# ZenHKD/ocr-vi-invoice

Measured on AMD Instinct MI355X. Metric: invoice images/sec end-to-end (det+rec), higher is better.
Workload: dtype f16x2

## Files before the change

include/ocrvi.h:

```cpp
#ifndef OCRVI_H
#define OCRVI_H

#include <stddef.h>
#include <stdint.h>

#ifdef __cplusplus
extern "C" {
#endif

#define OCRVI_OK 0
#define OCRVI_EINVAL (-1)
#define OCRVI_EHIP (-2)
#define OCRVI_ENOMEM (-3)
#define OCRVI_EBLOB (-4)
#define OCRVI_ERANGE (-5)

typedef enum { OCRVI_F32 = 0, OCRVI_BF16 = 1, OCRVI_F16 = 2, OCRVI_F16X2 = 3 } ocrvi_dtype;

const char* ocrvi_last_error(void);
int ocrvi_abi_version(void);

typedef struct ocrvi_det ocrvi_det;

typedef struct {
// ... 277 lines not shown
int ocrvi_test_gconv_plan(int dtype, int N, int C, int H, int W, int Co, int sh, int sw, int groups, int out_f32, int has_res, int n_cu,
                          int32_t plan[12]);
int ocrvi_test_conv3_halo_raw(int device, const float* x, const float* weight_host, const float* bias_host, int N, int C, int H, int W, int Co,
                              int act, void* out_raw, float* out);
int ocrvi_test_bneck_tail_raw(int device, const float* t1, const float* identity, const float* w2_host, const float* b2_host,
                              const float* w3_host, const float* b3_host, const float* w1_host, const float* b1_host, int N, int H, int W,
                              int no_phase_c, void* y_raw, void* t1n_raw, float* y_out, float* t1n_out);
int ocrvi_test_stem_pool_raw(int device, int dtype, const float* x, const float* weight_host, const float* bias_host, int N, int H, int W,
                             int fused, void* out_raw, float* out);
int ocrvi_test_halo_plan(int kind, int N, int C, int H, int W, int Co, int n_cu, int32_t plan[8]);
int ocrvi_test_stem_pool(int device, int dtype, const float* x, const float* weight_host, const float* bias_host, int N, int H, int W, int fused,
                         float* out, int iters, float* avg_ms);
int ocrvi_test_attention(int device, int dtype, const float* qkv, int B, int N, int heads, float* out, int iters,
                         float* avg_ms);

int ocrvi_test_mlp(int device, int dtype, float* x, const float* ln_g_host, const float* ln_b_host, const float* w1_host, const float* b1_host,
                   const float* w2_host, const float* b2_host, const float* next_g_host, const float* next_b_host, int want_xn, int M, int D,
                   float* xn_out, int iters, float* avg_ms);
int ocrvi_test_mlp_raw(int device, int dtype, float* x, const float* ln_g_host, const float* ln_b_host, const float* w1_host, const float* b1_host,
                       const float* w2_host, const float* b2_host, const float* next_g_host, const float* next_b_host, int M, int D, void* xn_raw,
                       float* xn_out, int iters, float* avg_ms);
int ocrvi_test_lin_x2(int device, const float* a, const float* weight_host, const float* bias_host, int M, int K, int N, int max_workgroups,
                      void* out_raw, float* out, int iters, float* avg_ms);
int ocrvi_test_pack_f16x2(const float* src, size_t n, void* dst, float* wscale);
int ocrvi_test_pack_stream(int kind, const float* w0, const float* w1, int d0, int d1, void* out, size_t cap, size_t* size, float scales[2]);
int ocrvi_test_swizzles(int32_t swz128_rows[64], int32_t swz_halo_rows[64]);
int ocrvi_test_persistent_grid(int ntile, int slots, int32_t* grid);

int ocrvi_test_layernorm(int device, int dtype, const float* x, int x_f32, int out_f32, const float* gamma_host, const float* beta_host,
                         int rows, int D, float* out);
int ocrvi_test_frm_vertical(int device, int dtype, const float* kv, const float* vq_host, int B, int H, int W, int D, float* out);
int ocrvi_test_asf(int device, int dtype, const float* p2, const float* p3, const float* p4, const float* p5, const float* w_host,
                   const float* b_host, int N, int H, int W, float* out);
int ocrvi_test_maxpool(int device, int dtype, const float* x, int N, int C, int H, int W, float* out);
int ocrvi_test_db_maps(int device, const float* bin_logits, const float* thresh_logits, float k, float* binary, float* thresh,
                       float* thresh_binary, size_t n);
int ocrvi_test_ctc_logsoftmax(int device, const float* logits, int ld, int B, int T, int C, float* log_probs, int32_t* argmax_ids);
int ocrvi_test_ctc_logsoftmax_conf(int device, const float* logits, int ld, int B, int T, int C, float* log_probs, int32_t* argmax_ids,
                                   float* best_lp);

int ocrvi_document_contour(const uint8_t* mask, int h, int w, int64_t stride, int32_t* quad , int32_t* found);
int ocrvi_document_contour_bits(const uint32_t* bits, int h, int w, int32_t* quad , int32_t* found);

#define OCRVI_DOC_AUTO 0
#define OCRVI_DOC_BRIGHT 1
#define OCRVI_DOC_DARK 2
// ... 31 lines not shown
```

ocr_vi_invoice_amd/_lib.py:

```python
from __future__ import annotations

import ctypes as C
import os
from typing import Optional

_HERE = os.path.dirname(os.path.abspath(__file__))
LIB_PATH = os.environ.get("OCRVI_LIB") or os.path.join(_HERE, "lib", "libocrvi.so")

OCRVI_F32, OCRVI_BF16, OCRVI_F16, OCRVI_F16X2 = 0, 1, 2, 3
DTYPES = {"f32": OCRVI_F32, "fp32": OCRVI_F32, "float32": OCRVI_F32, "bf16": OCRVI_BF16, "bfloat16": OCRVI_BF16,
          "f16": OCRVI_F16, "fp16": OCRVI_F16, "float16": OCRVI_F16,
          "f16x2": OCRVI_F16X2}
ABI_VERSION = 5

EXPORTS = [
    "ocrvi_last_error", "ocrvi_abi_version",
    "ocrvi_det_create", "ocrvi_det_destroy", "ocrvi_det_workspace_bytes", "ocrvi_det_forward", "ocrvi_det_debug_features",
    "ocrvi_rec_create", "ocrvi_rec_destroy", "ocrvi_rec_workspace_bytes", "ocrvi_rec_forward", "ocrvi_rec_debug_features",
    "ocrvi_ctc_greedy", "ocrvi_normalize_u8", "ocrvi_resize_u8", "ocrvi_crop_resize_normalize", "ocrvi_db_postprocess", "ocrvi_db_boxes_batch",
    "ocrvi_unclip_polygon", "ocrvi_db_components_workspace_bytes", "ocrvi_db_components", "ocrvi_db_boxes_batch_sparse",
    "ocrvi_test_deform_conv", "ocrvi_test_offset_conv", "ocrvi_test_conv", "ocrvi_test_gemm", "ocrvi_test_attention", "ocrvi_test_mlp", "ocrvi_test_stem_pool", "ocrvi_test_pack_f16x2",
    "ocrvi_prof_enable", "ocrvi_prof_reset", "ocrvi_prof_report",
    "ocrvi_det_status", "ocrvi_rec_status", "ocrvi_range_reset", "ocrvi_range_flag",
    "ocrvi_resize_normalize_pages", "ocrvi_crop_resize_normalize_pages", "ocrvi_db_boxes_pages",
# ... 4 lines not shown
    "ocrvi_test_deform_conv_res",
    "ocrvi_enhance_init", "ocrvi_enhance_tables", "ocrvi_enhance_workspace_bytes", "ocrvi_enhance_u8",
    "ocrvi_rgb_to_lab_u8", "ocrvi_lab_to_rgb_u8", "ocrvi_clahe_lab_u8", "ocrvi_nlm_lab_u8", "ocrvi_sharpen_u8",
    "ocrvi_min_area_quads", "ocrvi_quad_crops", "ocrvi_crop_quad_resize_normalize_pages", "ocrvi_crop_quad_resize_normalize",
    "ocrvi_jpeg_info", "ocrvi_jpeg_parse", "ocrvi_jpeg_table_entry", "ocrvi_jpeg_decode_pages",
    "ocrvi_test_conv_res", "ocrvi_test_db_tail",
    "ocrvi_db_target_jobs", "ocrvi_db_target_maps", "ocrvi_resize_normalize_pad_pages",
    "ocrvi_test_mlp_raw", "ocrvi_test_lin_x2", "ocrvi_test_pack_stream", "ocrvi_test_swizzles", "ocrvi_test_persistent_grid",
    "ocrvi_test_bneck_tail",
    "ocrvi_jpeg_quant_tables", "ocrvi_jpeg_encode_header", "ocrvi_jpeg_encode_sizes", "ocrvi_jpeg_encode_table_entry", "ocrvi_jpeg_encode_pages",
    "ocrvi_test_gemm_raw", "ocrvi_test_ring_plan",
    "ocrvi_overlay_segments", "ocrvi_overlay_pages",
    "ocrvi_test_deform_conv_raw", "ocrvi_test_dcn_plan",
    "ocrvi_test_conv_raw", "ocrvi_test_gconv_plan",
    "ocrvi_png_info", "ocrvi_png_parse", "ocrvi_png_table_entry", "ocrvi_png_plan", "ocrvi_png_decode_pages",
    "ocrvi_png_encode_sizes", "ocrvi_png_encode_table_entry", "ocrvi_png_encode_pages", "ocrvi_test_png_code_lengths",
    "ocrvi_document_contour", "ocrvi_document_contour_bits", "ocrvi_doc_working_size", "ocrvi_doc_mask_sizes", "ocrvi_doc_mask_pages",
    "ocrvi_doc_grey_u8", "ocrvi_doc_smooth_u8", "ocrvi_doc_histogram", "ocrvi_doc_otsu", "ocrvi_doc_mask_bits",
    "ocrvi_rec_forward_conf", "ocrvi_ctc_greedy_conf", "ocrvi_test_ctc_logsoftmax_conf",
    "ocrvi_test_conv3_halo_raw", "ocrvi_test_bneck_tail_raw", "ocrvi_test_stem_pool_raw", "ocrvi_test_halo_plan",
    "ocrvi_ctc_beam_workspace_bytes", "ocrvi_ctc_beam",
    "ocrvi_lm_build", "ocrvi_lm_score", "ocrvi_lm_create", "ocrvi_lm_destroy", "ocrvi_ctc_beam_lm_workspace_bytes", "ocrvi_ctc_beam_lm",
    "ocrvi_skew_sizes", "ocrvi_skew_scores_pages", "ocrvi_skew_edges_u8", "ocrvi_skew_scores", "ocrvi_skew_pick", "ocrvi_skew_quad",
]
PAGE_ENTRY = 4
DET_EVAL_RECORD_BYTES = 104
DET_EVAL_INT_SLOTS = ("tp", "fp", "fn", "positive_count", "negatives", "negative_count")
DET_EVAL_F64_SLOTS = ("pos_bce", "topk_bce", "dice_inter", "pred_mask", "gt_mask", "l1_num", "thresh_mask")
CTC_LOSS_MAX_TARGET = 1024
EDIT_DISTANCE_MAX_LEN = 2048
CTC_BEAM_MAX = 64
CTC_BEAM_MAX_T = 1024
LM_MAX_ORDER = 6
CLAHE_WORKSPACE_BYTES = 16384
ENHANCE_MIN_SIDE = 16
DB_TARGET_GT, DB_TARGET_MASK, DB_TARGET_THRESH = 0, 1, 2
DB_TARGET_JOB = 8
DB_TARGET_MAX_SIDE = 16384
JPEG_ENTRY = 64
PNG_ENTRY = 16
JPEG_ENC_ENTRY = 64
JPEG_HEADER_MAX = 640
PNG_ENC_ENTRY = 16
PNG_ENC_BLOCK = 16384
OVERLAY_SEG = 8
OVERLAY_PRIM = 8
# ... 79 lines not shown
    lib.ocrvi_four_point_transform.argtypes = [vp, vp, vp, i32p, i32p]
    lib.ocrvi_warp_perspective_u8.argtypes = [i32, vp, i32, i32, vp, vp, i32, i32, vp]
    lib.ocrvi_warp_perspective_pages.argtypes = [i32, vp, vp, vp, i32, vp]
    lib.ocrvi_db_boxes_pages.argtypes = [vp, i32, i32, i32, C.c_float, C.c_float, i32, C.c_float, C.c_float, vp, vp, vp, vp, vp,
                                         vp, i32, vp, vp, vp, i32, vp, vp, i32]
    lib.ocrvi_test_deform_conv.argtypes = [i32, i32, f32p, f32p, f32p, vp, vp, i32, i32, i32, i32, i32, i32, i32, f32p, i32,
                                           C.POINTER(C.c_float)]
    lib.ocrvi_test_deform_conv_res.argtypes = [i32, i32, f32p, f32p, f32p, vp, vp, f32p, i32, i32, i32, i32, i32, i32, i32, f32p, i32,
                                               C.POINTER(C.c_float)]
    lib.ocrvi_test_offset_conv.argtypes = [i32, i32, f32p, vp, vp, i32, i32, i32, i32, i32, f32p, i32, C.POINTER(C.c_float)]
    lib.ocrvi_test_conv.argtypes = [i32, i32, f32p, vp, vp, i32, i32, i32, i32, i32, i32, i32, i32, i32, i32, f32p, i32,
                                    C.POINTER(C.c_float)]
    lib.ocrvi_test_conv_res.argtypes = [i32, i32, f32p, vp, vp, f32p, i32, i32, i32, i32, i32, i32, i32, i32, f32p, i32, C.POINTER(C.c_float)]
    lib.ocrvi_test_bneck_tail.argtypes = [i32, f32p, f32p, vp, vp, vp, vp, vp, vp, i32, i32, i32, i32, f32p, f32p, i32, C.POINTER(C.c_float)]
    lib.ocrvi_test_db_tail.argtypes = [i32, i32, f32p, vp, vp, vp, vp, vp, vp, vp, vp, i32, i32, i32, i32, i32, f32p, f32p, i32,
                                       C.POINTER(C.c_float)]
    lib.ocrvi_test_gemm.argtypes = [i32, i32, f32p, vp, vp, f32p, i32, i32, i32, i32, i32, i32, f32p, i32, C.POINTER(C.c_float)]
    lib.ocrvi_test_gemm_raw.argtypes = [i32, i32, f32p, vp, vp, f32p, i32, i32, i32, i32, i32, i32, vp, f32p]
    lib.ocrvi_test_ring_plan.argtypes = [i32, i32, i32, i32, i32, i32, i32, i32, C.POINTER(C.c_int32)]
    lib.ocrvi_test_deform_conv_raw.argtypes = [i32, i32, f32p, f32p, f32p, vp, vp, f32p, i32, i32, i32, i32, i32, i32, i32, vp, f32p]
    lib.ocrvi_test_dcn_plan.argtypes = [i32, i32, i32, i32, i32, i32, i32, i32, C.POINTER(C.c_int32)]
    lib.ocrvi_test_conv_raw.argtypes = [i32, i32, f32p, vp, vp, f32p] + [i32] * 13 + [vp, f32p]
    lib.ocrvi_test_gconv_plan.argtypes = [i32] * 12 + [C.POINTER(C.c_int32)]
    lib.ocrvi_test_stem_pool.argtypes = [i32, i32, f32p, vp, vp, i32, i32, i32, i32, f32p, i32, C.POINTER(C.c_float)]
    lib.ocrvi_test_conv3_halo_raw.argtypes = [i32, f32p, vp, vp, i32, i32, i32, i32, i32, i32, vp, f32p]
    lib.ocrvi_test_bneck_tail_raw.argtypes = [i32, f32p, f32p, vp, vp, vp, vp, vp, vp, i32, i32, i32, i32, vp, vp, f32p, f32p]
    lib.ocrvi_test_stem_pool_raw.argtypes = [i32, i32, f32p, vp, vp, i32, i32, i32, i32, vp, f32p]
    lib.ocrvi_test_halo_plan.argtypes = [i32] * 7 + [C.POINTER(C.c_int32)]
    lib.ocrvi_test_attention.argtypes = [i32, i32, f32p, i32, i32, i32, f32p, i32, C.POINTER(C.c_float)]
    lib.ocrvi_test_mlp.argtypes = [i32, i32, f32p, vp, vp, vp, vp, vp, vp, vp, vp, i32, i32, i32, f32p, i32, C.POINTER(C.c_float)]
    lib.ocrvi_test_lin_x2.argtypes = [i32, f32p, vp, vp, i32, i32, i32, i32, vp, f32p, i32, C.POINTER(C.c_float)]
    lib.ocrvi_test_mlp_raw.argtypes = [i32, i32, f32p, vp, vp, vp, vp, vp, vp, vp, vp, i32, i32, vp, f32p, i32, C.POINTER(C.c_float)]
    lib.ocrvi_test_pack_f16x2.argtypes = [f32p, sz, vp, C.POINTER(C.c_float)]
    lib.ocrvi_test_pack_stream.argtypes = [i32, vp, vp, i32, i32, vp, sz, C.POINTER(sz), C.POINTER(C.c_float)]
    lib.ocrvi_test_swizzles.argtypes = [C.POINTER(C.c_int32), C.POINTER(C.c_int32)]
    lib.ocrvi_test_persistent_grid.argtypes = [i32, i32, C.POINTER(C.c_int32)]
    lib.ocrvi_test_layernorm.argtypes = [i32, i32, f32p, i32, i32, vp, vp, i32, i32, f32p]
    lib.ocrvi_test_frm_vertical.argtypes = [i32, i32, f32p, vp, i32, i32, i32, i32, f32p]
    lib.ocrvi_test_asf.argtypes = [i32, i32, f32p, f32p, f32p, f32p, vp, vp, i32, i32, i32, f32p]
    lib.ocrvi_test_maxpool.argtypes = [i32, i32, f32p, i32, i32, i32, i32, f32p]
    lib.ocrvi_test_db_maps.argtypes = [i32, f32p, f32p, C.c_float, f32p, f32p, f32p, sz]
    lib.ocrvi_test_ctc_logsoftmax.argtypes = [i32, f32p, i32, i32, i32, i32, f32p, i32p]
    lib.ocrvi_det_eval_workspace_bytes.argtypes = [i32, i32, i32, C.POINTER(sz)]
    lib.ocrvi_det_eval.argtypes = [i32, f32p, f32p, f32p, f32p, f32p, f32p, f32p, f32p, i32, i32, i32, C.c_double, vp, vp, sz, vp]
    lib.ocrvi_ctc_loss.argtypes = [i32, f32p, i32, i32, i32, i32p, i32, i32p, i32p, i32, vp, vp]
    lib.ocrvi_edit_distance.argtypes = [i32, i32p, i32, i32p, i32p, i32, i32p, i32, i32p, vp]
# ... 114 lines not shown
```

ocr_vi_invoice_amd/csrc/gconv32.h:

```cpp
#pragma once
#include "conv_gemm.h"

namespace ocrvi {

constexpr int GC_PS = 96;
constexpr int GC_TH = 4;
constexpr int GC_NBX = 5;

constexpr unsigned gc_hw_magic(int hw) { return 65536u / (unsigned)hw + 1; }
constexpr bool gc_hw_magic_exact() {
    for (int nbx = 1; nbx <= GC_NBX; ++nbx) {
        const int hw = 16 * nbx + 2;
        for (int pix = 0; pix < (GC_TH + 2) * hw; ++pix)
            if ((int)(((unsigned)pix * gc_hw_magic(hw)) >> 16) != pix / hw) return false;
    }
    return true;
}
static_assert(gc_hw_magic_exact(), "gconv32: the halo-index multiplication is not exact for every pixel of a (GC_TH + 2) x (16 GC_NBX + 2) tile");

template <typename T, bool F32O>
__global__ __launch_bounds__(256, 2) void gconv32_kernel(const ConvParams p, int TH, int nbx, int bands_y, int bands_x, unsigned hw_magic) {
    constexpr int PS = GC_PS, MB = (GC_TH * GC_NBX + 3) / 4;
    extern __shared__ __attribute__((aligned(16))) char smem[];
    const int tid = threadIdx.x, lane = tid & 63, wave = tid >> 6;
// ... 132 lines not shown
                if (F32O && p.res_mode == RES_SAME) {
                    const float4 rv = *(const float4*)((const float*)p.res + pix * p.ldr + ch);
                    v[nb][0] += rv.x; v[nb][1] += rv.y; v[nb][2] += rv.z; v[nb][3] += rv.w;
                }
                if (!p.res_post) activate(v[nb]);
                if (F32O) *(float4*)((float*)p.out + pix * p.ldo + p.out_coff + ch) = make_float4(v[nb][0], v[nb][1], v[nb][2], v[nb][3]);
            }
            if (!F32O) {
                union { T e[8]; uint4 u; } pk;
#pragma unroll
                for (int e = 0; e < 4; ++e) {
                    pk.e[e] = from_f32<T>(v[0][e]);
                    pk.e[4 + e] = from_f32<T>(v[1][e]);
                }
                *(uint4*)((T*)p.out + pix * p.ldo + p.out_coff + gp * 32 + 8 * g4) = pk.u;
            }
        }
        if (next >= ntile) break;
        tile = next;
        __syncthreads();
    }
}

static inline bool gconv32_eligible(const ConvParams& p, int amode, int esz) {
    static const bool on = !(getenv("OCRVI_GCONV32") && atoi(getenv("OCRVI_GCONV32")) == 0);
    if (!on || amode != AM_CONV3 || esz != 2 || p.groups < 2 || p.Cin_g != 32 || p.N_g != 32 || p.KH != 3) return false;
    if (p.SH != 1 || p.SW != 1 || p.PH != 1 || p.PW != 1 || p.H != p.OH || p.W != p.OW || p.store_mode != ST_NHWC) return false;
    if (p.Kp < 288 || p.Cin % 8 != 0 || p.cin_off % 8 != 0 || ((uintptr_t)p.x & 15) != 0 || ((uintptr_t)p.w & 15) != 0 || p.Kp % 8 != 0) return false;
    const int og = p.out_f32 ? 4 : 8;
    if (p.ldo % og != 0 || p.out_coff % og != 0 || ((uintptr_t)p.out & 15) != 0) return false;
    if (p.res_mode == RES_SAME) return p.out_f32 && p.res_f32 && p.ldr % 4 == 0 && ((uintptr_t)p.res & 15) == 0;
    return p.res_mode == RES_NONE;
}

struct Gconv32Plan {
    int th, nbx;
    int bands_y, bands_x;
    int ntile, grid_x;
    int tiles_min, tiles_max;
    int smem;
    unsigned hw_magic;
};
inline Gconv32Plan gconv32_plan(int n_img, int H, int W, int groups, int n_cu) {
    Gconv32Plan r;
    r.nbx = std::min(GC_NBX, cdiv(W, 16));
    r.th = H % 4 == 0 ? 4 : (H % 3 == 0 ? 3 : (H < 4 ? H : 4));
    r.bands_x = cdiv(W, 16 * r.nbx);
    r.bands_y = cdiv(H, r.th);
// ... 32 lines not shown
```

ocr_vi_invoice_amd/csrc/kernels.h:

```cpp
#pragma once
#include "common.h"

namespace ocrvi {

int k_nchw3_to_nhwc4_pad(int dtype, const float* x, void* y, int N, int H, int W, int pad_t, int pad_l, int Hp, int Wp, hipStream_t s);
int k_maxpool3x3s2(int dtype, const void* x, void* y, int N, int H, int W, int C, hipStream_t s);
bool stem_pool_eligible(int dtype, int cout, int Kp, int KH, int H, int W);
int k_stem_pool(int dtype, const void* xpad, const void* w, const float* bias, float wscale, void* y, int N, int H, int W, int Hp, int Wp,
                hipStream_t s);
struct StemPoolPlan {
    int tyN, txN, total;
    int grid;
    int tiles_min, tiles_max;
};
StemPoolPlan stem_pool_plan(int N, int H, int W, int n_cu);
int k_layernorm(int dtype, const void* x, int x_f32, void* out, int out_f32, const float* gamma, const float* beta, int rows, int D,
                hipStream_t s);
bool mlp_fused_eligible(int dtype, int D);
bool mlp_x2_eligible(int dtype, int D);
void pack_mlp_x2_stream(const float* w1, const float* w2, int D, std::vector<char>& out);
int k_mlp_x2(float* x, void* xn, const float* ln_g, const float* ln_b, const float* next_g, const float* next_b, const void* wstream, const float* b1,
             const float* b2, int M, int D, hipStream_t s);
void pack_mlp_stream(const float* w1, const float* w2, int D, int dtype, std::vector<char>& out);
bool lin_x2_eligible(int dtype, int K, int N);
void pack_lin_x2_stream(const float* w, int N, int K, std::vector<char>& out);
int k_lin_x2(const void* a, const void* wstream, const float* bias, void* out, int M, int K, int N, hipStream_t s, int max_workgroups = 0);
int k_mlp_fused(int dtype, float* x, void* xn, const float* ln_g, const float* ln_b, const float* next_g, const float* next_b, const void* wstream,
                const float* b1, const float* b2, int M, int D, hipStream_t s);
int k_cast_from_f32(int dtype, const float* x, void* y, size_t n, hipStream_t s);
int k_nhwc_to_nchw_f32(int dtype, const void* x, float* y, int N, int H, int W, int C, int ld, int coff, hipStream_t s);

int k_attention(int dtype, const void* qkv, void* out, int B, int N, int heads, hipStream_t s, void* scratch = nullptr);
size_t attention_scratch_bytes(int dtype, int B, int N, int heads);
int k_frm_vertical(int dtype, const void* kv, const float* vq, void* out, int B, int H, int W, int D, hipStream_t s);

int k_asf(int dtype, const void* p2, const void* p3, const void* p4, const void* p5, const float* w, const float* b, float* scratch, void* out,
          int N, int H, int W, hipStream_t s);
size_t asf_scratch_bytes(int N, int H, int W);
int k_db_maps(const float* bin_logits, const float* thresh_logits, float k, float* binary, float* thresh, float* thresh_binary, size_t n,
              hipStream_t s);

int k_ctc_logsoftmax_argmax(const float* logits, int ld, float* log_probs, int32_t* argmax_ids, int B, int T, int C, hipStream_t s);
int k_ctc_argmax_tbc(const float* log_probs, int32_t* argmax_ids, int B, int T, int C, hipStream_t s);
int k_ctc_collapse(const int32_t* argmax_ids, int32_t* ids, int32_t* lens, int B, int T, int blank, hipStream_t s);
int k_ctc_logsoftmax_argmax_conf(const float* logits, int ld, float* log_probs, int32_t* argmax_ids, float* best_lp, int B, int T, int C,
                                 hipStream_t s);
int k_ctc_argmax_tbc_conf(const float* log_probs, int32_t* argmax_ids, float* best_lp, int B, int T, int C, hipStream_t s);
int k_ctc_collapse_conf(const int32_t* argmax_ids, const float* best_lp, int32_t* ids, int32_t* lens, float* char_lp, int32_t* char_span, int B,
                        int T, int blank, hipStream_t s);
// ... 3 lines not shown
```

ocr_vi_invoice_amd/csrc/model.h:

```cpp
#pragma once
#include "conv_gemm.h"
#include "kernels.h"

namespace ocrvi {

struct DeviceStore {
    std::vector<void*> ptrs;
    ~DeviceStore() {
        for (void* p : ptrs) (void)hipFree(p);
    }
    int upload(const void* host, size_t bytes, void** out) {
        void* d = nullptr;
        OCRVI_HIP(hipMalloc(&d, bytes ? bytes : 16));
        ptrs.push_back(d);
        if (bytes) OCRVI_HIP(hipMemcpy(d, host, bytes, hipMemcpyHostToDevice));
        *out = d;
        return OCRVI_OK;
    }
    int upload_f32(const std::vector<float>& v, float** out) { return upload(v.data(), v.size() * 4, (void**)out); }
};

struct ConvLayer {
    void* w = nullptr;
    float* bias = nullptr;
// ... 26 lines not shown
    Arena arena;
    Runner(int dt, hipStream_t s, void* ws, size_t bytes) : dtype(dt), stream(s), arena(ws, bytes) {}
    bool dry() const { return arena.planning(); }
    size_t esz(bool f32) const { return f32 ? 4 : dtype_size(dtype); }
    Tensor alloc(int n, int h, int w, int c, bool f32 = false) {
        return wrap(arena.alloc((size_t)n * h * w * c * esz(f32)), n, h, w, c, f32);
    }
};

struct ConvOpts {
    int sh = 1, sw = 1, pad = 0;
    int act = ACT_NONE;
    const Tensor* res = nullptr;
    int res_mode = RES_NONE;
    int res_post = 0;
    int store_mode = ST_NHWC;
    const float* offs = nullptr;
    void* out2 = nullptr;
    int out_coff = 0;
    int cin_off = 0;
    int Hp = 0, Wp = 0;
};
int conv(Runner& r, const ConvLayer& L, const Tensor& x, const Tensor& y, const ConvOpts& o);


int finish_create(int dtype, RangeWatch& range);

template <typename Handle, typename Check, typename Run>
int plan_workspace(const char* what, const Handle* h, size_t* bytes, Check&& check, Run&& run) {
    OCRVI_CHECK(bytes, OCRVI_EINVAL, "%s: null out", what);
    OCRVI_TRY(check());
    Runner r(h->cfg.dtype, nullptr, nullptr, 0);
    OCRVI_TRY(run(r));
    *bytes = r.arena.peak + 256;
    return OCRVI_OK;
}

template <typename Handle, typename Check, typename Run>
int run_forward(const char* what, Handle* h, bool have_args, const char* args_msg, void* workspace, size_t workspace_bytes, void* stream,
                Check&& check, Run&& run) {
    OCRVI_TRY(check());
    OCRVI_CHECK(have_args, OCRVI_EINVAL, "%s: %s", what, args_msg);
    DeviceGuard dg(h->device);
    OCRVI_HIP(dg.err);
    Runner plan(h->cfg.dtype, nullptr, nullptr, 0);
    OCRVI_TRY(run(plan));
// ... 11 lines not shown
```

ocr_vi_invoice_amd/csrc/model_common.hip:

```cpp
#include "model.h"

#include "gemm_ring.h"

namespace ocrvi {

int upload_packed(DeviceStore& st, const PackedConv& pc, int amode, ConvLayer* L) {
    OCRVI_TRY(st.upload(pc.bytes.data(), pc.bytes.size(), &L->w));
    L->bias = nullptr;
    if (!pc.bias.empty()) OCRVI_TRY(st.upload_f32(pc.bias, &L->bias));
    L->Np = pc.Np; L->Kp = pc.Kp; L->N_g = pc.N_g; L->Cin_g = pc.Cin_g; L->groups = pc.groups; L->KH = pc.KH;
    L->amode = amode;
    L->wscale = pc.wscale;
    L->quartets = pc.quartets;
    return OCRVI_OK;
}

int load_conv(DeviceStore& st, const Blob& blob, const std::string& name, int cout, int cin_g, int k, int groups, int amode, int dtype,
              bool has_bias, ConvLayer* L, const float* extra_bias, bool halo) {
    const BlobTensor *w = nullptr, *b = nullptr;
    OCRVI_TRY(blob.get(name + ".w", cout, cin_g, k, k, &w));
    if (has_bias) OCRVI_TRY(blob.get(name + ".b", cout, 0, 0, 0, &b));
    std::vector<float> bias;
    if (b) bias.assign(b->data, b->data + cout);
    if (extra_bias) {
        if (bias.empty()) bias.assign(cout, 0.f);
        for (int i = 0; i < cout; ++i) bias[i] += extra_bias[i];
    }
    const int kk = k == 0 ? 1 : k;
    PackedConv pc = pack_conv(w->data, bias.empty() ? nullptr : bias.data(), cout, cin_g, kk, kk, groups, amode, dtype, halo);
    return upload_packed(st, pc, amode, L);
}

int load_vec(DeviceStore& st, const Blob& blob, const std::string& name, int n, float** out) {
    const BlobTensor* t = nullptr;
    OCRVI_TRY(blob.get(name, n, 0, 0, 0, &t));
    return st.upload(t->data, (size_t)n * 4, (void**)out);
}

int conv(Runner& r, const ConvLayer& L, const Tensor& x, const Tensor& y, const ConvOpts& o) {
    ConvParams p;
    p.x = x.p; p.w = L.w; p.bias = L.bias; p.out = y.p;
    p.n_img = x.n; p.H = x.h; p.W = x.w; p.Cin = x.c;
    p.KH = L.KH; p.SH = o.sh; p.SW = o.sw; p.PH = o.pad; p.PW = o.pad;
    p.Cin_g = L.Cin_g; p.cin_off = o.cin_off;
    p.N_g = L.N_g; p.Np = L.Np; p.Kp = L.Kp; p.groups = L.groups;
    p.store_mode = o.store_mode;
    p.wscale = L.wscale;
    p.w_quartets = L.quartets ? 1 : 0;
    if (o.store_mode == ST_SHUFFLE2) {
        p.OH = y.h / 2; p.OW = y.w / 2; p.shuffle_co = L.shuffle_co;
    } else if (o.store_mode == ST_DB_TAIL) {
        p.OH = y.h / 4; p.OW = y.w / 4; p.shuffle_co = L.shuffle_co; p.out2 = o.out2;
    } else if (o.store_mode == ST_DB_BIN) {
        p.OH = y.h / 4; p.OW = y.w / 4; p.shuffle_co = L.shuffle_co;
    } else {
        p.OH = y.h; p.OW = y.w;
    }
    p.M = x.n * p.OH * p.OW;
    p.ldo = o.store_mode == ST_DCN_OFFS ? 32 : y.c;
    p.out_coff = o.out_coff;
    p.out_f32 = y.f32 ? 1 : 0;
    p.act = o.act;
    p.res_post = o.res_post;
    if (o.res) {
        p.res = o.res->p; p.res_mode = o.res_mode; p.ldr = o.res->c; p.res_f32 = o.res->f32 ? 1 : 0;
    }
    p.offs = o.offs;
    p.Hp = o.Hp; p.Wp = o.Wp;
    OCRVI_CHECK(!x.f32 || r.dtype == OCRVI_F32, OCRVI_EINVAL, "conv: f32 activations fed to a %d-typed GEMM", r.dtype);
    if (L.amode != AM_ROWS) {
        const int k = L.amode == AM_CONV1 ? 1 : 3;
        const int eh = (x.h + 2 * o.pad - k) / o.sh + 1, ew = (x.w + 2 * o.pad - k) / o.sw + 1;
        OCRVI_CHECK(eh == p.OH && ew == p.OW, OCRVI_EINVAL, "conv: output %dx%d but expected %dx%d", p.OH, p.OW, eh, ew);
    }
    if (r.dry()) return OCRVI_OK;
    return launch_conv_dt(r.dtype, p, L.amode, r.stream);
}

int finish_create(int dtype, RangeWatch& range) {
    const void* zero_page;
    void* dump_page;
    OCRVI_TRY(ring_pages(&zero_page, &dump_page));
    if (dtype == OCRVI_F16X2) OCRVI_TRY(range.init());
    return OCRVI_OK;
}

}
```

ocr_vi_invoice_amd/csrc/rec_model.hip:

```cpp
#include <stdlib.h>
#include <string.h>

#include <algorithm>
#include <memory>

#include "model.h"

using namespace ocrvi;

namespace {
struct LNw { float *g = nullptr, *b = nullptr; };
struct MlpW {
    ConvLayer fc1, fc2;
    void* stream = nullptr;
    float *b1 = nullptr, *b2 = nullptr;
};
struct BlockW {
    bool local = false;
    LNw n1, n2;
    ConvLayer conv1, conv2;
    ConvLayer qkv, proj;
    void* qkv_lin = nullptr;
    MlpW mlp;
};
// ... 121 lines not shown
}

static int check_rec_shape(const ocrvi_rec* h, int B, int H, int W) {
    OCRVI_CHECK(h, OCRVI_EINVAL, "rec: null handle");
    OCRVI_CHECK(B > 0 && H > 0 && W > 0 && H % 16 == 0 && W % 4 == 0, OCRVI_EINVAL,
                "rec: input (B=%d,3,%d,%d) needs H %% 16 == 0 and W %% 4 == 0", B, H, W);
    const int tok = (H / 4) * (W / 4) / 2, tok_max = dtype_size(h->cfg.dtype) == 2 ? 1024 : 4096;
    OCRVI_CHECK(tok <= tok_max && H / 16 <= 8, OCRVI_EINVAL,
                "rec: %dx%d gives %d tokens in the first global-attention stage (at most %d in this mode) or more than 8 rows after the backbone", H, W, tok, tok_max);
    OCRVI_CHECK((size_t)B * (H / 2) * (W / 2) < ((size_t)1 << 23), OCRVI_EINVAL, "rec: batch of %d %dx%d crops too large for one call (chunk it)", B, H, W);
    return OCRVI_OK;
}

static int ln(Runner& r, const Tensor& x, const Tensor& y, const LNw& w) {
    if (r.dry()) return OCRVI_OK;
    return k_layernorm(r.dtype, x.p, x.f32, y.p, y.f32, w.g, w.b, (int)x.pixels(), x.c, r.stream);
}
static Tensor view(const Tensor& t, int n, int h, int w, int c) { return wrap(t.p, n, h, w, c, t.f32); }
static int linear(Runner& r, const ConvLayer& L, void* lin, const Tensor& x, const Tensor& y) {
    if (!lin) return conv(r, L, x, y, ConvOpts());
    if (r.dry()) return OCRVI_OK;
    return k_lin_x2(x.p, lin, L.bias, y.p, (int)x.pixels(), x.c, y.c, r.stream);
}
static int attention(Runner& r, const Tensor& qkv, const Tensor& out, int seqs, int len, int heads) {
    const size_t mk = r.arena.mark(), sb = attention_scratch_bytes(r.dtype, seqs, len, heads);
    void* asc = sb ? r.arena.alloc(sb) : nullptr;
    if (!r.dry()) OCRVI_TRY(k_attention(r.dtype, qkv.p, out.p, seqs, len, heads, r.stream, asc));
    r.arena.release(mk);
    return OCRVI_OK;
}

static const LNw kCast{};
static int mlp_block(Runner& r, const Tensor& x, const Tensor& xn, const Tensor& hb, const LNw& n, const MlpW& m, int d, const LNw* next = nullptr,
                     bool* xn_done = nullptr) {
    const int rows = (int)x.pixels();
    if (xn_done) *xn_done = false;
    if (m.stream) {
        if (xn_done) *xn_done = next != nullptr;
        if (r.dry()) return OCRVI_OK;
        return k_mlp_fused(r.dtype, (float*)x.p, next ? xn.p : nullptr, n.g, n.b, next ? next->g : nullptr, next ? next->b : nullptr, m.stream, m.b1, m.b2,
                           rows, d, r.stream);
    }
    OCRVI_TRY(ln(r, x, xn, n));
    ConvOpts o1;
    o1.act = ACT_GELU;
    OCRVI_TRY(conv(r, m.fc1, view(xn, rows, 1, 1, d), view(hb, rows, 1, 1, 4 * d), o1));
// ... 43 lines not shown
        ConvOpts o;
        o.sh = o.sw = 2; o.pad = 1; o.act = ACT_GELU; o.Hp = Hp; o.Wp = Wp;
        OCRVI_TRY(conv(r, h->stem1, xpad, s1, o));
    }
    int cur = 0;
    Tensor xs = wrap(X[cur], B, Hs, Ws, c.dims[0], true);
    {
        ConvOpts o;
        o.sh = o.sw = 2; o.pad = 1; o.act = ACT_GELU;
        OCRVI_TRY(conv(r, h->stem2, s1, xs, o));
    }
    for (int s = 0; s < 3; ++s) {
        const int d = c.dims[s];
        const int rows = B * Hs * Ws;
        const Tensor xn = wrap(XN, B, Hs, Ws, d, false), t1 = wrap(T1, B, Hs, Ws, d, false), big = wrap(BIG, rows, 1, 1, 4 * d, false);
        bool xn_ready = false;
        const int nblk = (int)h->blocks[s].size();
        for (int bi = 0; bi < nblk; ++bi) {
            const BlockW& bw = h->blocks[s][bi];
            if (!xn_ready) OCRVI_TRY(ln(r, xs, xn, bw.n1));
            if (bw.local) {
                ConvOpts o;
                o.pad = 1; o.act = ACT_GELU;
                OCRVI_TRY(conv(r, bw.conv1, xn, t1, o));
                o.res = &xs; o.res_mode = RES_SAME; o.res_post = 1;
                OCRVI_TRY(conv(r, bw.conv2, t1, xs, o));
            } else {
                ConvOpts o;
                OCRVI_TRY(linear(r, bw.qkv, bw.qkv_lin, view(xn, rows, 1, 1, d), view(big, rows, 1, 1, 3 * d)));
                OCRVI_TRY(attention(r, big, t1, B, Hs * Ws, d / 32));
                o.res = &xs; o.res_mode = RES_SAME;
                OCRVI_TRY(conv(r, bw.proj, view(t1, rows, 1, 1, d), view(xs, rows, 1, 1, d), o));
            }
            const LNw* next = bi + 1 < nblk ? &h->blocks[s][bi + 1].n1 : ((s < 2 && lowp) ? &kCast : nullptr);
            OCRVI_TRY(mlp_block(r, view(xs, rows, 1, 1, d), xn, big, bw.n2, bw.mlp, d, next, &xn_ready));
        }
        if (s < 2) {
            Tensor src = xn;
            if (lowp) {
                if (!xn_ready && !r.dry()) OCRVI_TRY(k_cast_from_f32(dt, (const float*)xs.p, xn.p, (size_t)rows * d, r.stream));
            } else {
                src = xs; src.f32 = false;
            }
            Tensor nx = wrap(X[cur ^ 1], B, Hs / 2, Ws, c.dims[s + 1], true);
            ConvOpts o;
            o.sh = 2; o.sw = 1; o.pad = 1;
            OCRVI_TRY(conv(r, h->merge[s], src, nx, o));
            xs = nx;
            cur ^= 1;
// ... 119 lines not shown
```

Baseline: 321.7.

## Add persistent halo-tiled f16x2 grouped 3x3 conv kernel for rec local blocks

Adds a dedicated f16x2 grouped 3x3 convolution kernel for the recognizer's local mixing blocks. It is persistent: each workgroup stages one 32-channel group's weights in shared memory once, loads swizzled halo tiles of the activations, and prefetches the next tile into registers while computing the current one. Bias, GELU/ReLU and an f32 residual add are fused into the epilogue. The aim is to cut the weight reloads and tile launch overhead of the generic grouped conv path. In exchange it brings a large amount of new kernel code, uses up to about 80KB of shared memory per workgroup which limits occupancy, and only takes calls that match strict shape and alignment checks.

```diff
diff --git a/include/ocrvi.h b/include/ocrvi.h
--- a/include/ocrvi.h
+++ b/include/ocrvi.h
@@ -323,6 +323,9 @@
                        float* xn_out, int iters, float* avg_ms);
 int ocrvi_test_lin_x2(int device, const float* a, const float* weight_host, const float* bias_host, int M, int K, int N, int max_workgroups,
                       void* out_raw, float* out, int iters, float* avg_ms);
+int ocrvi_test_gconv_x2(int device, const float* x, const float* weight_host, const float* bias_host, const float* res, int N, int C, int H, int W,
+                        int act, int res_post, int out_f32, int in_place, int max_workgroups, void* out_raw, float* out, int iters, float* avg_ms);
+int ocrvi_test_gconv_x2_plan(int N, int C, int H, int W, int n_cu, int max_workgroups, int32_t plan[10]);
 int ocrvi_test_pack_f16x2(const float* src, size_t n, void* dst, float* wscale);
 int ocrvi_test_pack_stream(int kind, const float* w0, const float* w1, int d0, int d1, void* out, size_t cap, size_t* size, float scales[2]);
 int ocrvi_test_swizzles(int32_t swz128_rows[64], int32_t swz_halo_rows[64]);
diff --git a/ocr_vi_invoice_amd/_lib.py b/ocr_vi_invoice_amd/_lib.py
--- a/ocr_vi_invoice_amd/_lib.py
+++ b/ocr_vi_invoice_amd/_lib.py
@@ -50,6 +50,7 @@
     "ocrvi_ctc_beam_workspace_bytes", "ocrvi_ctc_beam",
     "ocrvi_lm_build", "ocrvi_lm_score", "ocrvi_lm_create", "ocrvi_lm_destroy", "ocrvi_ctc_beam_lm_workspace_bytes", "ocrvi_ctc_beam_lm",
     "ocrvi_skew_sizes", "ocrvi_skew_scores_pages", "ocrvi_skew_edges_u8", "ocrvi_skew_scores", "ocrvi_skew_pick", "ocrvi_skew_quad",
+    "ocrvi_test_gconv_x2", "ocrvi_test_gconv_x2_plan",
 ]
 PAGE_ENTRY = 4
 DET_EVAL_RECORD_BYTES = 104
@@ -175,6 +176,8 @@
     lib.ocrvi_test_dcn_plan.argtypes = [i32, i32, i32, i32, i32, i32, i32, i32, C.POINTER(C.c_int32)]
     lib.ocrvi_test_conv_raw.argtypes = [i32, i32, f32p, vp, vp, f32p] + [i32] * 13 + [vp, f32p]
     lib.ocrvi_test_gconv_plan.argtypes = [i32] * 12 + [C.POINTER(C.c_int32)]
+    lib.ocrvi_test_gconv_x2.argtypes = [i32, f32p, vp, vp, f32p] + [i32] * 9 + [vp, f32p, i32, C.POINTER(C.c_float)]
+    lib.ocrvi_test_gconv_x2_plan.argtypes = [i32] * 6 + [C.POINTER(C.c_int32)]
     lib.ocrvi_test_stem_pool.argtypes = [i32, i32, f32p, vp, vp, i32, i32, i32, i32, f32p, i32, C.POINTER(C.c_float)]
     lib.ocrvi_test_conv3_halo_raw.argtypes = [i32, f32p, vp, vp, i32, i32, i32, i32, i32, i32, vp, f32p]
     lib.ocrvi_test_bneck_tail_raw.argtypes = [i32, f32p, f32p, vp, vp, vp, vp, vp, vp, i32, i32, i32, i32, vp, vp, f32p, f32p]
diff --git a/ocr_vi_invoice_amd/csrc/gconv32.h b/ocr_vi_invoice_amd/csrc/gconv32.h
--- a/ocr_vi_invoice_amd/csrc/gconv32.h
+++ b/ocr_vi_invoice_amd/csrc/gconv32.h
@@ -178,8 +178,13 @@
     }
 }
 
+static inline bool gconv32_on() {
+    static const bool on = !(getenv("OCRVI_GCONV32") && atoi(getenv("OCRVI_GCONV32")) == 0);
+    return on;
+}
+
 static inline bool gconv32_eligible(const ConvParams& p, int amode, int esz) {
-    static const bool on = !(getenv("OCRVI_GCONV32") && atoi(getenv("OCRVI_GCONV32")) == 0);
+    const bool on = gconv32_on();
     if (!on || amode != AM_CONV3 || esz != 2 || p.groups < 2 || p.Cin_g != 32 || p.N_g != 32 || p.KH != 3) return false;
     if (p.SH != 1 || p.SW != 1 || p.PH != 1 || p.PW != 1 || p.H != p.OH || p.W != p.OW || p.store_mode != ST_NHWC) return false;
     if (p.Kp < 288 || p.Cin % 8 != 0 || p.cin_off % 8 != 0 || ((uintptr_t)p.x & 15) != 0 || ((uintptr_t)p.w & 15) != 0 || p.Kp % 8 != 0) return false;
diff --git a/ocr_vi_invoice_amd/csrc/gconv_x2.hip b/ocr_vi_invoice_amd/csrc/gconv_x2.hip
--- /dev/null
+++ b/ocr_vi_invoice_amd/csrc/gconv_x2.hip
@@ -0,0 +1,271 @@
+#include <stdlib.h>
+
+#include "gconv32.h"
+#include "kernels.h"
+
+namespace ocrvi {
+OCRVI_RANGE_FLAG_TU()
+
+constexpr int GX_MAX_BH = 12;
+constexpr int GX_MAX_BLK = 12;
+constexpr int GX_MAX_NBX = 4;
+constexpr int GX_HALO_PIX = 288;
+constexpr int GX_W_BYTES = 9 * 32 * 128;
+
+static inline int gx_nbx(int bh, int W) {
+    int nbx = std::min(std::min(GX_MAX_BLK / bh, GX_MAX_NBX), cdiv(W, 16));
+    while (nbx > 1 && (bh + 2) * (16 * nbx + 2) > GX_HALO_PIX) --nbx;
+    return nbx;
+}
+constexpr bool gx_hw_magic_exact() {
+    for (int nbx = 1; nbx <= GX_MAX_NBX; ++nbx) {
+        const int hw = 16 * nbx + 2;
+        for (int pix = 0; pix < GX_HALO_PIX; ++pix)
+            if ((int)(((unsigned)pix * gc_hw_magic(hw)) >> 16) != pix / hw) return false;
+    }
+    return true;
+}
+static_assert(gx_hw_magic_exact(), "gconv_x2: the halo-index multiplication is not exact for every pixel of a tile");
+static_assert((GX_MAX_BH + 2) * 18 <= GX_HALO_PIX, "gconv_x2: a 12-row tile of one block does not fit the halo");
+
+template <bool F32O>
+__global__ __launch_bounds__(256, 2) void gconv_x2_kernel(const ConvParams p, int bh, int nbx, int bands_y, int bands_x, unsigned hw_magic) {
+    typedef f16x2_t T;
+    typedef Mma<T>::u4v U;
+    constexpr int MB = GX_MAX_BLK / 4;
+    constexpr int HPASS = GX_HALO_PIX * 8 / 256, WPASS = (32 * 36 + 255) / 256;
+    extern __shared__ __attribute__((aligned(16))) char smem[];
+    const int tid = threadIdx.x, lane = tid & 63;
+    const int wave = __builtin_amdgcn_readfirstlane(tid >> 6);
+    const int lr = lane & 15, g4 = lane >> 4;
+    const int TW = 16 * nbx, HW = TW + 2, HH = bh + 2;
+    char* const halo = smem;
+    char* const wl = smem + HH * HW * 128;
+    const int gp = (int)blockIdx.x % p.groups, G = (int)gridDim.x / p.groups;
+    const int ntile = p.n_img * bands_y * bands_x;
+    const char* const Xg = (const char*)p.x + (size_t)(p.cin_off + gp * 32) * 4;
+    const size_t pix_b = (size_t)p.Cin * 4;
+    uint4 hv[HPASS];
+    const int htotal = HH * HW * 8;
+    auto tile_origin = [&](int t, int& img, int& y0, int& x0) {
+        const int bx = t % bands_x;
+        t /= bands_x;
+        const int by = t % bands_y;
+        img = t / bands_y;
+        y0 = by * bh;
+        x0 = bx * TW;
+    };
+    auto fetch = [&](int t) {
+        int img, y0, x0;
+        tile_origin(t, img, y0, x0);
+        const char* X = Xg + (size_t)img * p.H * p.W * pix_b;
+#pragma unroll
+        for (int k = 0; k < HPASS; ++k) {
+            if (256 * k < htotal) {
+                const int i = min(tid + 256 * k, htotal - 1);
+                const int pix = i >> 3, c = i & 7;
+                const int hy = (int)(((unsigned)pix * hw_magic) >> 16), hx = pix - hy * HW;
+                const int iy = min(max(y0 + hy - 1, 0), p.H - 1), ix = min(max(x0 + hx - 1, 0), p.W - 1);
+                hv[k] = *(const uint4*)(X + ((size_t)iy * p.W + ix) * pix_b + c * 16);
+            }
+        }
+    };
+    auto stage = [&](int t) {
+        int img, y0, x0;
+        tile_origin(t, img, y0, x0);
+#pragma unroll
+        for (int k = 0; k < HPASS; ++k) {
+            const int i = tid + 256 * k;
+            if (i < htotal) {
+                const int pix = i >> 3, c = i & 7;
+                const int hy = (int)(((unsigned)pix * hw_magic) >> 16), hx = pix - hy * HW;
+                const int iy = y0 + hy - 1, ix = x0 + hx - 1;
+                const bool in = (unsigned)iy < (unsigned)p.H && (unsigned)ix < (unsigned)p.W;
+                *(uint4*)(halo + pix * 128 + ((c ^ swz_halo(pix)) << 4)) = in ? hv[k] : make_uint4(0, 0, 0, 0);
+            }
+        }
+    };
+    int tile = (int)blockIdx.x / p.groups;
+    if (tile >= ntile) return;
+    fetch(tile);
+    {
+        const char* Wg = (const char*)p.w + (size_t)gp * p.Np * p.Kp * 4;
+        uint4 wv[WPASS][2];
+#pragma unroll
+        for (int k = 0; k < WPASS; ++k) {
+            const int i = min(tid + 256 * k, 32 * 36 - 1);
+            const int n = i / 36, rem = i - n * 36, tap = rem >> 2, q = rem & 3;
+            const char* s = Wg + (size_t)n * p.Kp * 4 + tap * 128 + q * 32;
+            wv[k][0] = *(const uint4*)s;
+            wv[k][1] = *(const uint4*)(s + 16);
+        }
+#pragma unroll
+        for (int k = 0; k < WPASS; ++k) {
+            const int i = tid + 256 * k;
+            if (i < 32 * 36) {
+                const int n = i / 36, rem = i - n * 36, tap = rem >> 2, q = rem & 3;
+                const int row = tap * 32 + n, sw = swz_halo(row);
+                *(uint4*)(wl + row * 128 + (((2 * q) ^ sw) << 4)) = make_uint4(wv[k][0].x, wv[k][0].y, wv[k][1].x, wv[k][1].y);
+                *(uint4*)(wl + row * 128 + (((2 * q + 1) ^ sw) << 4)) = make_uint4(wv[k][0].z, wv[k][0].w, wv[k][1].z, wv[k][1].w);
+            }
+        }
+    }
+    stage(tile);
+    __syncthreads();
+    const int nblk = bh * nbx;
+    int pbase[MB], bty[MB], btb[MB];
+#pragma unroll
+    for (int m = 0; m < MB; ++m) {
+        const int mb = min(wave + 4 * m, nblk - 1);
+        bty[m] = mb / nbx;
+        btb[m] = mb - bty[m] * nbx;
+        pbase[m] = bty[m] * HW + btb[m] * 16 + lr;
+    }
+    const int wo = lr * 128 + (((2 * g4) ^ swz_halo(lr)) << 4);
+    float4 bias_r[2];
+#pragma unroll
+    for (int nb = 0; nb < 2; ++nb) bias_r[nb] = p.bias ? *(const float4*)(p.bias + gp * 32 + nb * 16 + 4 * g4) : make_float4(0.f, 0.f, 0.f, 0.f);
+    auto activate = [&](float (&v)[4]) {
+        if (p.act == ACT_RELU) {
+#pragma unroll
+            for (int e = 0; e < 4; ++e) v[e] = fmaxf(v[e], 0.f);
+        } else if (p.act == ACT_GELU) {
+#pragma unroll
+            for (int e = 0; e < 4; ++e) v[e] = gelu_erf(v[e]);
+        }
+    };
+    unsigned long long bad = 0;
+    constexpr bool EARLY = F32O;
+    int next = tile + G;
+    if (EARLY && next < ntile) fetch(next);
+    for (;;) {
+        if (!EARLY && next < ntile) fetch(next);
+        int img, y0, x0;
+        tile_origin(tile, img, y0, x0);
+        bool ok[MB];
+        size_t opix[MB];
+#pragma unroll
+        for (int m = 0; m < MB; ++m) {
+            const int y = y0 + bty[m], x = x0 + btb[m] * 16 + lr;
+            ok[m] = wave + 4 * m < nblk && y < p.H && x < p.W;
+            opix[m] = ok[m] ? ((size_t)img * p.H + y) * p.W + x : 0;
+        }
+        float4 rres[MB][2];
+        if constexpr (F32O) {
+#pragma unroll
+            for (int m = 0; m < MB; ++m)
+#pragma unroll
+                for (int nb = 0; nb < 2; ++nb)
+                    rres[m][nb] = ok[m] ? *(const float4*)((const float*)p.res + opix[m] * p.ldr + gp * 32 + nb * 16 + 4 * g4) : make_float4(0.f, 0.f, 0.f, 0.f);
+        }
+        f32x4 acc[MB][2];
+#pragma unroll
+        for (int m = 0; m < MB; ++m) acc[m][0] = acc[m][1] = (f32x4){0.f, 0.f, 0.f, 0.f};
+#pragma unroll
+        for (int tap = 0; tap < 9; ++tap) {
+            const int r = tap / 3, s = tap - r * 3;
+            U wH[2], wL[2];
+#pragma unroll
+            for (int nb = 0; nb < 2; ++nb) {
+                const char* wr = wl + (tap * 32 + nb * 16) * 128 + wo;
+                wH[nb] = Mma<T>::as_u4v(*(const uint4*)wr);
+                wL[nb] = Mma<T>::as_u4v(*(const uint4*)(wl + (tap * 32 + nb * 16) * 128 + (wo ^ 16)));
+            }
+#pragma unroll
+            for (int m = 0; m < MB; ++m) {
+                const int pp = pbase[m] + r * HW + s;
+                const int o = pp * 128 + (((2 * g4) ^ swz_halo(pp)) << 4);
+                U xH, xL;
+                Mma<T>::regroup(*(const uint4*)(halo + o), *(const uint4*)(halo + (o ^ 16)), xH, xL);
+                Mma<T>::three(wH[0], wL[0], xH, xL, acc[m][0]);
+                Mma<T>::three(wH[1], wL[1], xH, xL, acc[m][1]);
+            }
+        }
+        __syncthreads();
+        const int after = next + G;
+        if (next < ntile) {
+            stage(next);
+            if (EARLY && after < ntile) fetch(after);
+        }
+#pragma unroll
+        for (int m = 0; m < MB; ++m) {
+#pragma unroll
+            for (int nb = 0; nb < 2; ++nb) {
+                const int ch = gp * 32 + nb * 16 + 4 * g4;
+                float v[4] = {unscale<T>(acc[m][nb][0], p.wscale) + bias_r[nb].x, unscale<T>(acc[m][nb][1], p.wscale) + bias_r[nb].y,
+                              unscale<T>(acc[m][nb][2], p.wscale) + bias_r[nb].z, unscale<T>(acc[m][nb][3], p.wscale) + bias_r[nb].w};
+                activate(v);
+                if constexpr (F32O) {
+                    const float4 rv = rres[m][nb];
+                    if (ok[m])
+                        *(float4*)((float*)p.out + opix[m] * p.ldo + p.out_coff + ch) = make_float4(v[0] + rv.x, v[1] + rv.y, v[2] + rv.z, v[3] + rv.w);
+                } else {
+                    bad |= f16x2_out_of_range(v) & __builtin_amdgcn_ballot_w64(ok[m]);
+                    if (ok[m]) *(uint4*)((char*)p.out + (opix[m] * p.ldo + p.out_coff + ch) * 4) = Chunk<T>::pack(v);
+                }
+            }
+        }
+        if (next >= ntile) break;
+        tile = next;
+        next = after;
+        __syncthreads();
+    }
+    if constexpr (!F32O) f16x2_raise(bad);
+}
+
+GconvX2Plan gconv_x2_plan(int n_img, int H, int W, int groups, int n_cu, int max_workgroups) {
+    GconvX2Plan r;
+    r.bh = std::min(H, GX_MAX_BH);
+    r.nbx = gx_nbx(r.bh, W);
+    r.bands_y = cdiv(H, r.bh);
+    r.bands_x = cdiv(W, 16 * r.nbx);
+    r.ntile = n_img * r.bands_y * r.bands_x;
+    int slots = std::max(1, 2 * n_cu / groups);
+    if (max_workgroups > 0) slots = std::min(slots, max_workgroups);
+    r.grid_x = persistent_grid(r.ntile, slots);
+    r.tiles_min = r.ntile / r.grid_x;
+    r.tiles_max = cdiv(r.ntile, r.grid_x);
+    r.smem = (r.bh + 2) * (16 * r.nbx + 2) * 128 + GX_W_BYTES;
+    return r;
+}
+
+static bool gconv_x2_takes(const ConvParams& p, int dtype) {
+    if (dtype != OCRVI_F16X2 || p.groups < 2 || p.Cin_g != 32 || p.N_g != 32 || p.Np != 32 || p.KH != 3 || p.w_quartets) return false;
+    if (p.SH != 1 || p.SW != 1 || p.PH != 1 || p.PW != 1 || p.H != p.OH || p.W != p.OW || p.H < 1 || p.W < 1 || p.store_mode != ST_NHWC) return false;
+    if (p.Kp < 288 || p.Kp % 4 != 0 || p.Cin % 4 != 0 || p.cin_off % 4 != 0 || p.cin_off + p.groups * 32 > p.Cin) return false;
+    if (!p.x || !p.w || !p.out || ((uintptr_t)p.x & 15) != 0 || ((uintptr_t)p.w & 15) != 0 || ((uintptr_t)p.out & 15) != 0) return false;
+    if (p.bias && ((uintptr_t)p.bias & 15) != 0) return false;
+    if (p.ldo % 4 != 0 || p.out_coff % 4 != 0 || p.out_coff + p.groups * 32 > p.ldo) return false;
+    if (p.act != ACT_NONE && p.act != ACT_RELU && p.act != ACT_GELU) return false;
+    if ((size_t)p.n_img * p.H * p.W >= ((size_t)1 << 23)) return false;
+    if (p.out_f32)
+        return p.res_mode == RES_SAME && p.res && p.res_f32 && p.res_post && p.ldr % 4 == 0 && p.groups * 32 <= p.ldr && ((uintptr_t)p.res & 15) == 0;
+    return p.res_mode == RES_NONE;
+}
+bool gconv_x2_eligible(const ConvParams& p, int dtype) { return gconv32_on() && gconv_x2_takes(p, dtype); }
+
+int k_gconv_x2(const ConvParams& p, hipStream_t stream, int max_workgroups) {
+    OCRVI_CHECK(gconv_x2_takes(p, OCRVI_F16X2), OCRVI_EINVAL, "gconv_x2: not a grouped 3x3 call this kernel takes (Cin_g %d, N_g %d, out_f32 %d, res %d)",
+                p.Cin_g, p.N_g, p.out_f32, p.res_mode);
+    int n_cu = 0;
+    OCRVI_TRY(device_cus(&n_cu));
+    const GconvX2Plan pl = gconv_x2_plan(p.n_img, p.H, p.W, p.groups, n_cu, max_workgroups);
+    const double px = (double)p.n_img * p.H * p.W, ch = 32.0 * p.groups;
+    char tag[64];
+    snprintf(tag, sizeof(tag), "gconv_x2_f16x2 M%d g%d %s", p.n_img * p.H * p.W, p.groups, p.out_f32 ? "res_f32" : "f16x2");
+    ProfScope ps(tag, 2.0 * px * ch * 288.0, px * ch * 4.0 + ch * 288.0 * 4.0 + px * ch * 4.0 + (p.out_f32 ? px * ch * 4.0 : 0.0), stream);
+    const dim3 grid(pl.grid_x * p.groups);
+    if (p.out_f32) {
+        auto k = gconv_x2_kernel<true>;
+        OCRVI_TRY(ensure_max_smem((const void*)k, 80 * 1024));
+        hipLaunchKernelGGL(k, grid, dim3(256), pl.smem, stream, p, pl.bh, pl.nbx, pl.bands_y, pl.bands_x, gc_hw_magic(16 * pl.nbx + 2));
+    } else {
+        auto k = gconv_x2_kernel<false>;
+        OCRVI_TRY(ensure_max_smem((const void*)k, 80 * 1024));
+        hipLaunchKernelGGL(k, grid, dim3(256), pl.smem, stream, p, pl.bh, pl.nbx, pl.bands_y, pl.bands_x, gc_hw_magic(16 * pl.nbx + 2));
+    }
+    OCRVI_HIP(hipGetLastError());
+    return OCRVI_OK;
+}
+
+}
diff --git a/ocr_vi_invoice_amd/csrc/kernels.h b/ocr_vi_invoice_amd/csrc/kernels.h
--- a/ocr_vi_invoice_amd/csrc/kernels.h
+++ b/ocr_vi_invoice_amd/csrc/kernels.h
@@ -25,6 +25,17 @@
 bool lin_x2_eligible(int dtype, int K, int N);
 void pack_lin_x2_stream(const float* w, int N, int K, std::vector<char>& out);
 int k_lin_x2(const void* a, const void* wstream, const float* bias, void* out, int M, int K, int N, hipStream_t s, int max_workgroups = 0);
+struct ConvParams;
+struct GconvX2Plan {
+    int bh, nbx;
+    int bands_y, bands_x;
+    int ntile, grid_x;
+    int tiles_min, tiles_max;
+    int smem;
+};
+GconvX2Plan gconv_x2_plan(int n_img, int H, int W, int groups, int n_cu, int max_workgroups = 0);
+bool gconv_x2_eligible(const ConvParams& p, int dtype);
+int k_gconv_x2(const ConvParams& p, hipStream_t s, int max_workgroups = 0);
 int k_mlp_fused(int dtype, float* x, void* xn, const float* ln_g, const float* ln_b, const float* next_g, const float* next_b, const void* wstream,
                 const float* b1, const float* b2, int M, int D, hipStream_t s);
 int k_cast_from_f32(int dtype, const float* x, void* y, size_t n, hipStream_t s);
diff --git a/ocr_vi_invoice_amd/csrc/model.h b/ocr_vi_invoice_amd/csrc/model.h
--- a/ocr_vi_invoice_amd/csrc/model.h
+++ b/ocr_vi_invoice_amd/csrc/model.h
@@ -72,6 +72,8 @@
     int Hp = 0, Wp = 0;
 };
 int conv(Runner& r, const ConvLayer& L, const Tensor& x, const Tensor& y, const ConvOpts& o);
+ConvParams fill_conv_params(const ConvLayer& L, const Tensor& x, const Tensor& y, const ConvOpts& o);
+int check_conv_shapes(const Runner& r, const ConvLayer& L, const Tensor& x, const ConvParams& p, const ConvOpts& o);
 
 
 int finish_create(int dtype, RangeWatch& range);
diff --git a/ocr_vi_invoice_amd/csrc/model_common.hip b/ocr_vi_invoice_amd/csrc/model_common.hip
--- a/ocr_vi_invoice_amd/csrc/model_common.hip
+++ b/ocr_vi_invoice_amd/csrc/model_common.hip
@@ -37,7 +37,7 @@
     return st.upload(t->data, (size_t)n * 4, (void**)out);
 }
 
-int conv(Runner& r, const ConvLayer& L, const Tensor& x, const Tensor& y, const ConvOpts& o) {
+ConvParams fill_conv_params(const ConvLayer& L, const Tensor& x, const Tensor& y, const ConvOpts& o) {
     ConvParams p;
     p.x = x.p; p.w = L.w; p.bias = L.bias; p.out = y.p;
     p.n_img = x.n; p.H = x.h; p.W = x.w; p.Cin = x.c;
@@ -67,12 +67,22 @@
     }
     p.offs = o.offs;
     p.Hp = o.Hp; p.Wp = o.Wp;
+    return p;
+}
+
+int check_conv_shapes(const Runner& r, const ConvLayer& L, const Tensor& x, const ConvParams& p, const ConvOpts& o) {
     OCRVI_CHECK(!x.f32 || r.dtype == OCRVI_F32, OCRVI_EINVAL, "conv: f32 activations fed to a %d-typed GEMM", r.dtype);
     if (L.amode != AM_ROWS) {
         const int k = L.amode == AM_CONV1 ? 1 : 3;
         const int eh = (x.h + 2 * o.pad - k) / o.sh + 1, ew = (x.w + 2 * o.pad - k) / o.sw + 1;
         OCRVI_CHECK(eh == p.OH && ew == p.OW, OCRVI_EINVAL, "conv: output %dx%d but expected %dx%d", p.OH, p.OW, eh, ew);
     }
+    return OCRVI_OK;
+}
+
+int conv(Runner& r, const ConvLayer& L, const Tensor& x, const Tensor& y, const ConvOpts& o) {
+    const ConvParams p = fill_conv_params(L, x, y, o);
+    OCRVI_TRY(check_conv_shapes(r, L, x, p, o));
     if (r.dry()) return OCRVI_OK;
     return launch_conv_dt(r.dtype, p, L.amode, r.stream);
 }
diff --git a/ocr_vi_invoice_amd/csrc/rec_model.hip b/ocr_vi_invoice_amd/csrc/rec_model.hip
--- a/ocr_vi_invoice_amd/csrc/rec_model.hip
+++ b/ocr_vi_invoice_amd/csrc/rec_model.hip
@@ -167,6 +167,16 @@
     if (r.dry()) return OCRVI_OK;
     return k_lin_x2(x.p, lin, L.bias, y.p, (int)x.pixels(), x.c, y.c, r.stream);
 }
+static int local_conv(Runner& r, const ConvLayer& L, const Tensor& x, const Tensor& y, const ConvOpts& o) {
+    if (r.dtype == OCRVI_F16X2 && L.amode == AM_CONV3) {
+        const ConvParams p = fill_conv_params(L, x, y, o);
+        if (gconv_x2_eligible(p, r.dtype)) {
+            OCRVI_TRY(check_conv_shapes(r, L, x, p, o));
+            return r.dry() ? OCRVI_OK : k_gconv_x2(p, r.stream);
+        }
+    }
+    return conv(r, L, x, y, o);
+}
 static int attention(Runner& r, const Tensor& qkv, const Tensor& out, int seqs, int len, int heads) {
     const size_t mk = r.arena.mark(), sb = attention_scratch_bytes(r.dtype, seqs, len, heads);
     void* asc = sb ? r.arena.alloc(sb) : nullptr;
@@ -256,9 +266,9 @@
             if (bw.local) {
                 ConvOpts o;
                 o.pad = 1; o.act = ACT_GELU;
-                OCRVI_TRY(conv(r, bw.conv1, xn, t1, o));
+                OCRVI_TRY(local_conv(r, bw.conv1, xn, t1, o));
                 o.res = &xs; o.res_mode = RES_SAME; o.res_post = 1;
-                OCRVI_TRY(conv(r, bw.conv2, t1, xs, o));
+                OCRVI_TRY(local_conv(r, bw.conv2, t1, xs, o));
             } else {
                 ConvOpts o;
                 OCRVI_TRY(linear(r, bw.qkv, bw.qkv_lin, view(xn, rows, 1, 1, d), view(big, rows, 1, 1, 3 * d)));
```

New measurement: 326.4, median of 6. +1.4%, better.
